# ZeayW/Multimodal-fusion-based-Pre-routing-Timing-Prediction-

Hardware: AMD Instinct MI355X
Metric: train-step samples/sec (higher is better)
Workload: dtype bf16; 1 GPU; config B: 8 designs/step/GPU, 65536-node netlist, 64 levels, 256x256 tile, 1350 endpoints/design, UNet(max), bf16 operands / fp32 accumulate on the MFMA-bound contractions; U-Net activations and their gradients stored bf16, netlist tensors, statistics, parameters and gradients fp32; nodes=65536, levels=64, tile=256, endpoints_per_design=1350, cone_pruning=False, parallelism=dp1 (designs sharded, one all-reduce of the flat gradient per step), launch=one HIP graph replay per step (Adam inside)

## Files before the change

multimodal-fusion-based-pre-routing-timing-prediction-_amd/csrc/unet16_conv.hip:

```cpp
#include <type_traits>
#include "unet16.h"

namespace mmft {

struct U16PackDesc {
  const float* w;
  u16* out;
  int rows, K;
  int taps;
  int mode;
  int Rsrc, Ksrc;
};

__global__ void __launch_bounds__(256) u16_pack_kernel(const U16PackDesc* __restrict__ descs, long long* __restrict__ counters,
                                                       int ncounters, long long inc) {
  if (counters && blockIdx.x == 0 && blockIdx.y == 0 && (int)threadIdx.x < ncounters) counters[threadIdx.x] += inc;
  const U16PackDesc d = descs[blockIdx.y];
  const int mode = d.mode & 3, KW = (d.mode & 4) ? 8 : 4, G = KW / 4;
  const int KB = d.K / (4 * KW), MB = d.rows / 16;
  const long long items = (long long)MB * d.taps * KB * 64 * G;
  for (long long e = (long long)blockIdx.x * 256 + threadIdx.x; e < items; e += (long long)gridDim.x * 256) {
    const int g = (int)(e % G);
    const int lane = (int)((e / G) & 63);
    long long f = e / (64 * G);
    const int kb = (int)(f % KB);
    f /= KB;
    const int t = (int)(f % d.taps), mb = (int)(f / d.taps);
    const int r = lane & 15, q = lane >> 4;
    const int row = mb * 16 + r;
    float v[4];
#pragma unroll
    for (int j = 0; j < 4; ++j) {
      const int k = kb * 4 * KW + KW * q + 4 * g + j;
      float x = 0.f;
      if (row < d.Rsrc && k < d.Ksrc) {
        if (mode == 0) x = d.w[((long long)row * d.taps + t) * d.Ksrc + k];
        else if (mode == 1) x = d.w[((long long)k * d.taps + (d.taps - 1 - t)) * d.Rsrc + row];
        else x = d.w[(long long)k * d.Rsrc + row];
      }
      v[j] = x;
    }
    *reinterpret_cast<s16x4*>(d.out + e * 4) = pack_bf16x4(v[0], v[1], v[2], v[3]);
  }
}

typedef __bf16 u16_bf16x8 __attribute__((ext_vector_type(8)));
typedef short u16_s16x8 __attribute__((ext_vector_type(8)));

struct U16ConvArgs {
  const void* x;
  const u16* wpk;
  u16* y;
  float* stats;
  int N, H, W, CO;
  int tiles_x, tiles_y, tiles;
  const float* gamma;
  const float* beta;
  const float* rmean;
  const float* rvar;
  float eps;
  int lda;
  u16* pooled;
  int pool_mode;
};

template <int CI, int TH, int TW>
struct U16ConvCfg {
  static constexpr bool K32 = CI >= 32;
  static constexpr int XR = TH + 2, XC = TW + 2, PIX = CI + (K32 ? 16 : 8);
  static constexpr int XS_BYTES = XR * XC * PIX * 2;
  static constexpr int RED_BYTES = 4 * 2 * 32 * 4;
  static constexpr int LDS_BYTES = XS_BYTES + RED_BYTES;
};

template <int CI, int COB, int TH, int TW, bool RGB, bool EVAL = false>
__global__ void __launch_bounds__(256) u16_conv3x3_kernel(U16ConvArgs a) {
  using C = U16ConvCfg<CI, TH, TW>;
  constexpr int XR = C::XR, XC = C::XC, PIX = C::PIX, MB = COB / 16;
  constexpr bool K32 = C::K32;
  constexpr int KC = K32 ? 32 : 16, NCH = CI / KC;
  constexpr int STEPS = TH * TW / 16, SPR = TW / 16, SPW = STEPS / 4;
  static_assert(TW % 16 == 0 && CI % 16 == 0 && COB % 16 == 0 && STEPS % 4 == 0 && (!RGB || CI == 16), "granularity");
  static_assert(!EVAL || (SPR <= 4 && (4 / SPR) * SPW == TH && SPW % 2 == 0), "eval epilogue: a wave owns SPW consecutive rows");
  extern __shared__ __attribute__((aligned(16))) unsigned char smem[];
  u16* xs = reinterpret_cast<u16*>(smem);
  float* red = reinterpret_cast<float*>(smem + C::XS_BYTES);
  const int tid = threadIdx.x, lane = tid & 63, wave = tid >> 6;
  const int r = lane & 15, q = lane >> 4;
  const int mb0 = blockIdx.y * MB, co0 = mb0 * 16;
  const f32x4 zero = {0.f, 0.f, 0.f, 0.f};
  auto strip = [&](int s, int& row, int& c0) {
    if constexpr (EVAL) {
      row = (wave / SPR) * SPW + s;
      c0 = (wave % SPR) * 16;
    } else {
      const int st = wave + 4 * s;
      row = st / SPR;
      c0 = (st % SPR) * 16;
    }
  };

  typedef typename std::conditional<K32, u16_bf16x8, s16x4>::type wfrag_t;
  wfrag_t wf[9][MB];
  auto load_weights = [&](int ch) {
#pragma unroll
    for (int t = 0; t < 9; ++t)
#pragma unroll
      for (int m = 0; m < MB; ++m)
        wf[t][m] = *reinterpret_cast<const wfrag_t*>(a.wpk + ((((long long)(mb0 + m) * 9 + t) * NCH + ch) * 64 + lane) * (KC / 4));
  };
  if constexpr (NCH == 1) load_weights(0);

  constexpr int XG = RGB ? 1 : CI / 8, XI = XR * XC * XG, NX = (XI + 255) / 256;
  if constexpr (RGB) {
    for (int e = tid; e < XR * XC * PIX / 4; e += 256) reinterpret_cast<s16x4*>(xs)[e] = s16x4{0, 0, 0, 0};
    __syncthreads();
  }
  u32x4 xr[NX];
  auto request = [&](int tile) {
    const int tx = tile % a.tiles_x, ty = (tile / a.tiles_x) % a.tiles_y, img = tile / (a.tiles_x * a.tiles_y);
    const int x0 = tx * TW, y0 = ty * TH;
    const long long img0 = (long long)img * a.H;
#pragma unroll
    for (int k = 0; k < NX; ++k) {
      const int it = tid + k * 256;
      const int cg = it % XG, col = (it / XG) % XC, row = it / (XG * XC);
      const int yy = y0 - 1 + row, xx = x0 - 1 + col;
      const bool ok = it < XI && yy >= 0 && yy < a.H && xx >= 0 && xx < a.W;
      const long long pix = (img0 + (ok ? yy : y0)) * a.W + (ok ? xx : x0);
      u32x4 v = {0u, 0u, 0u, 0u};
      if constexpr (RGB) {
        const float* src = reinterpret_cast<const float*>(a.x) + pix * 3;
        const s16x4 p = pack_bf16x4(src[0], src[1], src[2], 0.f);
        const u32x2 pp = as_u32x2(p);
        v[0] = pp[0];
        v[1] = pp[1];
      } else {
        v = *reinterpret_cast<const u32x4*>(reinterpret_cast<const u16*>(a.x) + pix * CI + cg * 8);
      }
      const u32x4 z4 = {0u, 0u, 0u, 0u};
      xr[k] = ok ? v : z4;
    }
  };
  auto deposit = [&]() {
#pragma unroll
    for (int k = 0; k < NX; ++k) {
      const int it = tid + k * 256;
      if (it < XI) {
        if constexpr (RGB) {
          u32x2 p = {xr[k][0], xr[k][1]};
          *reinterpret_cast<u32x2*>(xs + it * PIX) = p;
        } else {
          *reinterpret_cast<u32x4*>(xs + (it / XG) * PIX + (it % XG) * 8) = xr[k];
        }
      }
    }
  };

  float sc[EVAL ? MB : 1][4], sh[EVAL ? MB : 1][4];
  if constexpr (EVAL) {
#pragma unroll
    for (int m = 0; m < MB; ++m)
#pragma unroll
      for (int j = 0; j < 4; ++j) {
        const int c = co0 + m * 16 + 4 * q + j;
        const float rv = a.rvar[c];
        sc[m][j] = bn_frozen_scale(a.gamma[c], rv, a.eps);
        sh[m][j] = __fmaf_rn(-a.rmean[c], sc[m][j], a.beta[c]);
      }
  }

  if ((int)blockIdx.x < a.tiles) request(blockIdx.x);
  for (int tile = blockIdx.x; tile < a.tiles; tile += gridDim.x) {
    deposit();
    __syncthreads();
    if (tile + (int)gridDim.x < a.tiles) request(tile + gridDim.x);
    const int tx = tile % a.tiles_x, ty = (tile / a.tiles_x) % a.tiles_y, img = tile / (a.tiles_x * a.tiles_y);
    const int x0 = tx * TW, y0 = ty * TH;
    f32x4 acc[SPW][MB];
#pragma unroll
    for (int s = 0; s < SPW; ++s)
#pragma unroll
      for (int m = 0; m < MB; ++m) acc[s][m] = zero;
#pragma unroll 1
    for (int ch = 0; ch < NCH; ++ch) {
      if constexpr (NCH > 1) load_weights(ch);
#pragma unroll
      for (int s = 0; s < SPW; ++s) {
        int row, c0;
        strip(s, row, c0);
#pragma unroll
        for (int ky = 0; ky < 3; ++ky)
#pragma unroll
          for (int kx = 0; kx < 3; ++kx)
          {
            const u16* xp = xs + ((row + ky) * XC + c0 + r + kx) * PIX + ch * KC + (KC / 4) * q;
            if constexpr (K32) {
              const u16_bf16x8 xf = *reinterpret_cast<const u16_bf16x8*>(xp);
#pragma unroll
              for (int m = 0; m < MB; ++m) acc[s][m] = __builtin_amdgcn_mfma_f32_16x16x32_bf16(wf[ky * 3 + kx][m], xf, acc[s][m], 0, 0, 0);
            } else {
              const s16x4 xf = *reinterpret_cast<const s16x4*>(xp);
#pragma unroll
              for (int m = 0; m < MB; ++m) acc[s][m] = mfma_bf16_k16(wf[ky * 3 + kx][m], xf, acc[s][m]);
            }
          }
      }
    }
    if constexpr (EVAL) {
      u32x2 pk[SPW][MB];
#pragma unroll
      for (int s = 0; s < SPW; ++s) {
        int row, c0;
        strip(s, row, c0);
        const int yy = y0 + row, xx = x0 + c0 + r;
        const bool valid = yy < a.H && xx < a.W;
        u16* out = a.y + (((long long)img * a.H + yy) * a.W + xx) * a.lda + co0;
#pragma unroll
        for (int m = 0; m < MB; ++m) {
          float v[4];
#pragma unroll
          for (int j = 0; j < 4; ++j) {
            const float t = bn_pre(acc[s][m][j], sc[m][j], sh[m][j]);
            v[j] = t > 0.f ? t : 0.f;
          }
          const s16x4 p4 = pack_bf16x4(v[0], v[1], v[2], v[3]);
          if (valid) *reinterpret_cast<s16x4*>(out + m * 16 + 4 * q) = p4;
          pk[s][m] = as_u32x2(p4);
        }
      }
      if (a.pooled) {
        const int H2 = a.H / 2, W2 = a.W / 2;
        int row0, c0;
        strip(0, row0, c0);
        const int xx = x0 + c0 + r;
#pragma unroll
        for (int s = 0; s < SPW; s += 2) {
          const int yy = y0 + row0 + s;
          const bool store = (r & 1) == 0 && yy < a.H && xx < a.W;
          u16* out = a.pooled + (((long long)img * H2 + yy / 2) * W2 + xx / 2) * a.CO + co0;
#pragma unroll
          for (int m = 0; m < MB; ++m) {
            u32x2 nb0, nb1;
#pragma unroll
            for (int i = 0; i < 2; ++i) {
              nb0[i] = __shfl_xor(pk[s][m][i], 1, 64);
              nb1[i] = __shfl_xor(pk[s + 1][m][i], 1, 64);
            }
            float f00[4], f01[4], f10[4], f11[4], o[4];
            unpack4(pk[s][m], f00);
            unpack4(nb0, f01);
            unpack4(pk[s + 1][m], f10);
            unpack4(nb1, f11);
#pragma unroll
            for (int j = 0; j < 4; ++j) {
              if (a.pool_mode == MMFT_POOL_MAX) o[j] = fmaxf(fmaxf(f00[j], f01[j]), fmaxf(f10[j], f11[j]));
              else o[j] = (((f00[j] + f01[j]) + f10[j]) + f11[j]) * 0.25f;
            }
            if (store) *reinterpret_cast<s16x4*>(out + m * 16 + 4 * q) = pack_bf16x4(o[0], o[1], o[2], o[3]);
          }
        }
      }
      __syncthreads();
      continue;
    }
    float sm[MB][4], sq[MB][4];
#pragma unroll
    for (int m = 0; m < MB; ++m)
#pragma unroll
      for (int j = 0; j < 4; ++j) sm[m][j] = sq[m][j] = 0.f;
#pragma unroll
    for (int s = 0; s < SPW; ++s) {
      int row, c0;
      strip(s, row, c0);
      const int yy = y0 + row, xx = x0 + c0 + r;
      const bool valid = yy < a.H && xx < a.W;
      u16* out = a.y + (((long long)img * a.H + yy) * a.W + xx) * a.CO + co0;
#pragma unroll
      for (int m = 0; m < MB; ++m) {
        const s16x4 pk = pack_bf16x4(acc[s][m]);
        if (valid) *reinterpret_cast<s16x4*>(out + m * 16 + 4 * q) = pk;
        if (a.stats) {
#pragma unroll
          for (int j = 0; j < 4; ++j) {
            const float v = valid ? bf2f((unsigned)(unsigned short)pk[j]) : 0.f;
            sm[m][j] += v;
            sq[m][j] = __fmaf_rn(v, v, sq[m][j]);
          }
        }
      }
    }
    if (a.stats) {
#pragma unroll
      for (int m = 0; m < MB; ++m)
#pragma unroll
        for (int j = 0; j < 4; ++j) {
          float s1 = sm[m][j], s2 = sq[m][j];
#pragma unroll
          for (int o = 1; o < 16; o <<= 1) {
            s1 += __shfl_xor(s1, o, 64);
            s2 += __shfl_xor(s2, o, 64);
          }
          if (r == 0) {
            red[(wave * 2 + 0) * 32 + m * 16 + 4 * q + j] = s1;
            red[(wave * 2 + 1) * 32 + m * 16 + 4 * q + j] = s2;
          }
        }
    }
    __syncthreads();
    if (a.stats && tid < 2 * COB) {
      const int which = tid / COB, c = tid % COB;
      const float t = ((red[(0 * 2 + which) * 32 + c] + red[(1 * 2 + which) * 32 + c]) + red[(2 * 2 + which) * 32 + c]) +
                      red[(3 * 2 + which) * 32 + c];
      a.stats[((long long)tile * 2 + which) * a.CO + co0 + c] = t;
    }
  }
}

struct U16WgradArgs {
  const void* x;
  const u16* dy;
  float* slabs;
  int N, H, W, CI, CO;
  int tiles_x, tiles_y, tiles;
};

constexpr int u16_tr_pitch(int ch) { return ch == 16 ? 16 : 48; }

template <int CIB, int COB, int TH, int TW>
struct U16WgradCfg {
  static constexpr int XR = TH + 2, XC = TW + 2, PIXX = u16_tr_pitch(CIB), PIXD = u16_tr_pitch(COB);
  static constexpr int XS_BYTES = XR * XC * PIXX * 2, DS_BYTES = TH * TW * PIXD * 2;
  static constexpr int LDS_BYTES = XS_BYTES + DS_BYTES;
};

typedef __attribute__((address_space(3))) s16x4 lds_s16x4;
__device__ __forceinline__ s16x4 lds_tr_read(const u16* p) {
  return __builtin_amdgcn_ds_read_tr16_b64_v4i16((lds_s16x4*)p);
}

__device__ __forceinline__ u16_bf16x8 join8(s16x4 lo, s16x4 hi) {
  u16_s16x8 v = {lo[0], lo[1], lo[2], lo[3], hi[0], hi[1], hi[2], hi[3]};
  return __builtin_bit_cast(u16_bf16x8, v);
}

template <int CIB, int COB, int TH, int TW, bool RGB>
__global__ void __launch_bounds__(256) u16_conv3x3_wgrad_kernel(U16WgradArgs a) {
  using C = U16WgradCfg<CIB, COB, TH, TW>;
  constexpr int XR = C::XR, XC = C::XC, PIXX = C::PIXX, PIXD = C::PIXD, CB = CIB / 16, MB = COB / 16;
  constexpr int UNITS = 9 * CB, UM = (UNITS + 3) / 4;
  constexpr int SPT = TW / 32, STEPS = TH * SPT;
  static_assert(TW % 32 == 0 && CIB % 16 == 0 && COB % 16 == 0 && (!RGB || CIB == 16), "granularity");
  extern __shared__ __attribute__((aligned(16))) unsigned char smem[];
  u16* xs = reinterpret_cast<u16*>(smem);
  u16* ds = reinterpret_cast<u16*>(smem + C::XS_BYTES);
  const int tid = threadIdx.x, lane = tid & 63, wave = __builtin_amdgcn_readfirstlane(tid >> 6);
  const int nci = RGB ? 1 : a.CI / CIB;
  const int co0 = ((int)blockIdx.y / nci) * COB, ci0 = ((int)blockIdx.y % nci) * CIB;
  const f32x4 zero = {0.f, 0.f, 0.f, 0.f};
  const int tr_pix = 4 * (lane >> 4) + ((lane >> 2) & 3), tr_ch = 4 * (lane & 3);

  f32x4 acc[MB][UM];
#pragma unroll
  for (int m = 0; m < MB; ++m)
#pragma unroll
    for (int i = 0; i < UM; ++i) acc[m][i] = zero;

  constexpr int XG = RGB ? 1 : CIB / 8, XI = XR * XC * XG, NX = (XI + 255) / 256;
  constexpr int DG = COB / 8, DI = TH * TW * DG, ND = (DI + 255) / 256;
  if constexpr (RGB) {
    for (int e = tid; e < XR * XC * PIXX / 4; e += 256) reinterpret_cast<s16x4*>(xs)[e] = s16x4{0, 0, 0, 0};
    __syncthreads();
  }
  u32x4 xr[NX], dr[ND];
  auto request = [&](int tile) {
    const int tx = tile % a.tiles_x, ty = (tile / a.tiles_x) % a.tiles_y, img = tile / (a.tiles_x * a.tiles_y);
    const int x0 = tx * TW, y0 = ty * TH;
    const long long img0 = (long long)img * a.H;
    const u32x4 z4 = {0u, 0u, 0u, 0u};
#pragma unroll
    for (int k = 0; k < NX; ++k) {
      const int it = tid + k * 256;
      const int cg = it % XG, col = (it / XG) % XC, row = it / (XG * XC);
      const int yy = y0 - 1 + row, xx = x0 - 1 + col;
      const bool ok = it < XI && yy >= 0 && yy < a.H && xx >= 0 && xx < a.W;
      const long long pix = (img0 + (ok ? yy : y0)) * a.W + (ok ? xx : x0);
      u32x4 v = z4;
      if constexpr (RGB) {
        const float* src = reinterpret_cast<const float*>(a.x) + pix * 3;
        const u32x2 pp = as_u32x2(pack_bf16x4(src[0], src[1], src[2], 0.f));
        v[0] = pp[0];
        v[1] = pp[1];
      } else {
        v = *reinterpret_cast<const u32x4*>(reinterpret_cast<const u16*>(a.x) + pix * a.CI + ci0 + cg * 8);
      }
      xr[k] = ok ? v : z4;
    }
#pragma unroll
    for (int k = 0; k < ND; ++k) {
      const int it = tid + k * 256;
      const int cg = it % DG, col = (it / DG) % TW, row = it / (DG * TW);
      const int yy = y0 + row, xx = x0 + col;
      const bool ok = it < DI && yy < a.H && xx < a.W;
      const long long pix = (img0 + (ok ? yy : y0)) * a.W + (ok ? xx : x0);
      const u32x4 v = *reinterpret_cast<const u32x4*>(a.dy + pix * a.CO + co0 + cg * 8);
      dr[k] = ok ? v : z4;
    }
  };
  auto deposit = [&]() {
#pragma unroll
    for (int k = 0; k < NX; ++k) {
      const int it = tid + k * 256;
      if (it < XI) {
        if constexpr (RGB) {
          u32x2 p = {xr[k][0], xr[k][1]};
          *reinterpret_cast<u32x2*>(xs + it * PIXX) = p;
        } else {
          *reinterpret_cast<u32x4*>(xs + (it / XG) * PIXX + (it % XG) * 8) = xr[k];
        }
      }
    }
#pragma unroll
    for (int k = 0; k < ND; ++k) {
      const int it = tid + k * 256;
      if (it < DI) *reinterpret_cast<u32x4*>(ds + (it / DG) * PIXD + (it % DG) * 8) = dr[k];
    }
  };

  if ((int)blockIdx.x < a.tiles) request(blockIdx.x);
  for (int tile = blockIdx.x; tile < a.tiles; tile += gridDim.x) {
    deposit();
    __syncthreads();
    if (tile + (int)gridDim.x < a.tiles) request(tile + gridDim.x);
#pragma unroll 2
    for (int st = 0; st < STEPS; ++st) {
      const int row = st / SPT, c0 = (st % SPT) * 32;
      u16_bf16x8 af[MB];
      const u16* dbase = ds + (row * TW + c0 + tr_pix) * PIXD + tr_ch;
#pragma unroll
      for (int m = 0; m < MB; ++m) af[m] = join8(lds_tr_read(dbase + m * 16), lds_tr_read(dbase + 16 * PIXD + m * 16));
#pragma unroll
      for (int i = 0; i < UM; ++i) {
        const int u = wave + 4 * i;
        if (u < UNITS) {
          const int t = u / CB, c = u % CB, ky = t / 3, kx = t % 3;
          const u16* xb = xs + ((row + ky) * XC + c0 + kx + tr_pix) * PIXX + c * 16 + tr_ch;
          const u16_bf16x8 bfr = join8(lds_tr_read(xb), lds_tr_read(xb + 16 * PIXX));
#pragma unroll
          for (int m = 0; m < MB; ++m) acc[m][i] = __builtin_amdgcn_mfma_f32_16x16x32_bf16(af[m], bfr, acc[m][i], 0, 0, 0);
        }
      }
    }
    __syncthreads();
  }

  const int r = lane & 15, q = lane >> 4;
  const int CIs = RGB ? 3 : a.CI;
  float* out = a.slabs + (long long)blockIdx.x * ((long long)a.CO * 9 * CIs);
#pragma unroll
  for (int i = 0; i < UM; ++i) {
    const int u = wave + 4 * i;
    if (u < UNITS) {
      const int t = u / CB, c = u % CB;
#pragma unroll
      for (int m = 0; m < MB; ++m)
#pragma unroll
        for (int j = 0; j < 4; ++j) {
          const int co = co0 + m * 16 + 4 * q + j, ci = c * 16 + r;
          if (!RGB || ci < 3) out[((long long)co * 9 + t) * CIs + ci0 + ci] = acc[m][i][j];
        }
    }
  }
}

static inline void u16_tile_shape(int W, int* th, int* tw) {
  *tw = W >= 64 ? 64 : 32;
  *th = 256 / *tw;
}

template <int CI, int COB, int TH, int TW, bool RGB, bool EVAL = false>
static int u16_conv_launch_t(const U16ConvArgs& a, int grid_x, hipStream_t st, double flops, double bytes) {
  using C = U16ConvCfg<CI, TH, TW>;
  static DynLdsOnce once;
  int rc = ensure_dyn_lds(once, reinterpret_cast<const void*>(&u16_conv3x3_kernel<CI, COB, TH, TW, RGB, EVAL>), C::LDS_BYTES, "u16_conv3x3");
  if (rc) return rc;
  static char name[64];
  if (!name[0])
    snprintf(name, sizeof(name), EVAL ? "u16_conv3x3_eval_kernel<%d,%d,%dx%d%s>" : "u16_conv3x3_kernel<%d,%d,%dx%d%s>", RGB ? 3 : CI, COB,
             TH, TW, a.stats ? "" : "");
  MMFT_LAUNCH_LDS(name, flops, bytes, (u16_conv3x3_kernel<CI, COB, TH, TW, RGB, EVAL>), dim3(grid_x, a.CO / COB), dim3(256),
                  C::LDS_BYTES, st, a);
  return check_launch(EVAL ? "u16_conv3x3_eval" : "u16_conv3x3");
}

template <bool EVAL>
static int u16_conv_dispatch(U16ConvArgs& a, int rgb_f32, int Ci, hipStream_t st, double flops, double bytes) {
  int th, tw;
  u16_tile_shape(a.W, &th, &tw);
  a.tiles_x = (a.W + tw - 1) / tw;
  a.tiles_y = (a.H + th - 1) / th;
  a.tiles = a.N * a.tiles_x * a.tiles_y;
  const int cob = a.CO % 32 == 0 ? 32 : 16, gy = a.CO / cob;
  int cap = 2048 / gy;
  const int gx = a.tiles < cap ? a.tiles : cap;
#define U16_CONV(CIV, COBV, RGBV)                                                                           \
  (tw == 64 ? u16_conv_launch_t<CIV, COBV, 4, 64, RGBV, EVAL>(a, gx, st, flops, bytes)                      \
            : u16_conv_launch_t<CIV, COBV, 8, 32, RGBV, EVAL>(a, gx, st, flops, bytes))
  if (rgb_f32) return U16_CONV(16, 16, true);
  if (cob == 16) {
    if (Ci == 16) return U16_CONV(16, 16, false);
    if (Ci == 32) return U16_CONV(32, 16, false);
    if (Ci == 64) return U16_CONV(64, 16, false);
    return U16_CONV(128, 16, false);
  }
  if (Ci == 16) return U16_CONV(16, 32, false);
  if (Ci == 32) return U16_CONV(32, 32, false);
  if (Ci == 64) return U16_CONV(64, 32, false);
  return U16_CONV(128, 32, false);
#undef U16_CONV
}

template <int CIB, int COB, int TH, int TW, bool RGB>
static int u16_wgrad_launch_t(const U16WgradArgs& a, int grid_x, int grid_y, hipStream_t st, double flops, double bytes) {
  using C = U16WgradCfg<CIB, COB, TH, TW>;
  static DynLdsOnce once;
  int rc = ensure_dyn_lds(once, reinterpret_cast<const void*>(&u16_conv3x3_wgrad_kernel<CIB, COB, TH, TW, RGB>), C::LDS_BYTES,
                          "u16_conv3x3_wgrad");
  if (rc) return rc;
  static char name[64];
  if (!name[0]) snprintf(name, sizeof(name), "u16_conv3x3_wgrad_kernel<%d,%d,%dx%d>", RGB ? 3 : CIB, COB, TH, TW);
  MMFT_LAUNCH_LDS(name, flops, bytes, (u16_conv3x3_wgrad_kernel<CIB, COB, TH, TW, RGB>), dim3(grid_x, grid_y),
                  dim3(256), C::LDS_BYTES, st, a);
  return check_launch("u16_conv3x3_wgrad");
}

static inline bool u16_channels_ok(int c) { return c == 16 || c == 32 || c == 64 || c == 128; }

static inline int u16_wgrad_grid_x(int tiles, int grid_y) {
  int cap = 512 / grid_y;
  if (cap < 8) cap = 8;
  int g = (tiles + 1) / 2;
  if (g > cap) g = cap;
  return g < 1 ? 1 : g;
}

}

using namespace mmft;

extern "C" {

int mmft_u16_pack_weights(const void* descs, int n, long long max_frag_lanes, long long* counters, int ncounters, long long inc,
                          int device, void* stream) {
  MMFT_REQUIRE(descs && n > 0 && max_frag_lanes > 0 && ncounters >= 0 && ncounters <= 256, "u16_pack_weights: bad arguments");
  DeviceGuard dg(device);
  long long gx = (max_frag_lanes + 255) / 256;
  if (gx > 64) gx = 64;
  MMFT_LAUNCH("u16_pack_kernel", 0.0, 6.0 * 4.0 * max_frag_lanes * n / 2, u16_pack_kernel, dim3((int)gx, n), dim3(256), (hipStream_t)stream,
              reinterpret_cast<const U16PackDesc*>(descs), counters, ncounters, inc);
  return check_launch("u16_pack_weights");
}

int mmft_u16_pack_desc_bytes(void) { return (int)sizeof(U16PackDesc); }

int mmft_u16_conv_tiles(int N, int H, int W, int* per_image) {
  int th, tw;
  u16_tile_shape(W, &th, &tw);
  const int t = ((H + th - 1) / th) * ((W + tw - 1) / tw);
  if (per_image) *per_image = t;
  return N * t;
}

int mmft_u16_conv3x3(const void* x, int rgb_f32, const void* wpk, void* y, float* stats, int N, int H, int W, int Ci, int Co,
                     int device, void* stream) {
  MMFT_REQUIRE(x && wpk && y && N > 0 && H > 0 && W > 0, "u16_conv3x3: bad arguments");
  MMFT_REQUIRE(u16_channels_ok(Co) && (rgb_f32 ? (Ci == 3 && Co == 16) : u16_channels_ok(Ci)),
               "u16_conv3x3: channels must be 16 / 32 / 64 / 128 (or the 3 -> 16 RGB layer)");
  MMFT_REQUIRE(aligned16(x) && aligned16(wpk) && aligned16(y), "u16_conv3x3: 16-byte alignment");
  DeviceGuard dg(device);
  U16ConvArgs a{x, reinterpret_cast<const u16*>(wpk), reinterpret_cast<u16*>(y), stats, N, H, W, Co};
  const double flops = 2.0 * N * H * W * Co * 9.0 * Ci;
  const double bytes = (rgb_f32 ? 4.0 : 2.0) * N * H * W * Ci + 2.0 * N * H * W * Co + 2.0 * Co * 9 * Ci;
  return u16_conv_dispatch<false>(a, rgb_f32, Ci, (hipStream_t)stream, flops, bytes);
}

int mmft_u16_conv3x3_eval(const void* x, int rgb_f32, const void* wpk, const float* gamma, const float* beta, const float* running_mean,
                          const float* running_var, float eps, void* a, int lda, void* pooled, int pool_mode, int N, int H, int W,
                          int Ci, int Co, int device, void* stream) {
  MMFT_REQUIRE(x && wpk && a && gamma && beta && running_mean && running_var && N > 0 && H > 0 && W > 0 && eps >= 0.f,
               "u16_conv3x3_eval: bad arguments");
  MMFT_REQUIRE(u16_channels_ok(Co) && (rgb_f32 ? (Ci == 3 && Co == 16) : u16_channels_ok(Ci)),
               "u16_conv3x3_eval: channels must be 16 / 32 / 64 / 128 (or the 3 -> 16 RGB layer)");
  MMFT_REQUIRE(lda >= Co && lda % 8 == 0, "u16_conv3x3_eval: the pixel pitch must hold Co channels and be a multiple of 8");
  MMFT_REQUIRE(!pooled || (H % 2 == 0 && W % 2 == 0 && (pool_mode == MMFT_POOL_MAX || pool_mode == MMFT_POOL_AVG)),
               "u16_conv3x3_eval: pooling needs even H, W and a pooling mode");
  MMFT_REQUIRE(aligned16(x) && aligned16(wpk) && aligned16(a) && (!pooled || aligned16(pooled)), "u16_conv3x3_eval: 16-byte alignment");
  DeviceGuard dg(device);
  U16ConvArgs p{x, reinterpret_cast<const u16*>(wpk), reinterpret_cast<u16*>(a), nullptr, N, H, W, Co};
  p.gamma = gamma;
  p.beta = beta;
  p.rmean = running_mean;
  p.rvar = running_var;
  p.eps = eps;
  p.lda = lda;
  p.pooled = reinterpret_cast<u16*>(pooled);
  p.pool_mode = pool_mode;
  const double flops = 2.0 * N * H * W * Co * 9.0 * Ci;
  const double bytes = (rgb_f32 ? 4.0 : 2.0) * N * H * W * Ci + 2.0 * N * H * W * Co * (pooled ? 1.25 : 1.0) + 2.0 * Co * 9 * Ci;
  return u16_conv_dispatch<true>(p, rgb_f32, Ci, (hipStream_t)stream, flops, bytes);
}

long long mmft_u16_conv3x3_wgrad_workspace_bytes(int N, int H, int W, int Ci, int Co) {
  int th, tw;
  u16_tile_shape(W, &th, &tw);
  const int tiles = N * ((H + th - 1) / th) * ((W + tw - 1) / tw);
  const int cib = Ci == 3 ? 16 : (Ci % 32 == 0 ? 32 : 16), cob = Co % 32 == 0 ? 32 : 16;
  const int gy = (Co / cob) * (Ci == 3 ? 1 : Ci / cib);
  return (long long)u16_wgrad_grid_x(tiles, gy) * Co * 9 * Ci * 4;
}

int mmft_u16_conv3x3_wgrad_slabs(int N, int H, int W, int Ci, int Co) {
  return (int)(mmft_u16_conv3x3_wgrad_workspace_bytes(N, H, W, Ci, Co) / ((long long)Co * 9 * Ci * 4));
}

int mmft_u16_conv3x3_wgrad(const void* x, int rgb_f32, const void* dy, float* dw, int accumulate, int N, int H, int W, int Ci,
                           int Co, float* workspace, long long workspace_bytes, int device, void* stream) {
  MMFT_REQUIRE(x && dy && N > 0 && H > 0 && W > 0, "u16_conv3x3_wgrad: bad arguments");
  MMFT_REQUIRE(u16_channels_ok(Co) && (rgb_f32 ? (Ci == 3 && Co == 16) : u16_channels_ok(Ci)),
               "u16_conv3x3_wgrad: channels must be 16 / 32 / 64 / 128 (or the 3 -> 16 RGB layer)");
  MMFT_REQUIRE(workspace && workspace_bytes >= mmft_u16_conv3x3_wgrad_workspace_bytes(N, H, W, Ci, Co) && aligned16(workspace) &&
                   aligned16(x) && aligned16(dy) && (!dw || aligned16(dw)),
               "u16_conv3x3_wgrad: workspace too small or operands not 16-byte aligned");
  DeviceGuard dg(device);
  hipStream_t st = (hipStream_t)stream;
  int th, tw;
  u16_tile_shape(W, &th, &tw);
  U16WgradArgs a{x, reinterpret_cast<const u16*>(dy), workspace, N, H, W, Ci, Co, (W + tw - 1) / tw, (H + th - 1) / th, 0};
  a.tiles = N * a.tiles_x * a.tiles_y;
  const int cib = rgb_f32 ? 16 : (Ci % 32 == 0 ? 32 : 16), cob = Co % 32 == 0 ? 32 : 16;
  const int gy = (Co / cob) * (rgb_f32 ? 1 : Ci / cib);
  const int gx = u16_wgrad_grid_x(a.tiles, gy);
  const double flops = 2.0 * N * H * W * Co * 9.0 * Ci;
  const double bytes = (rgb_f32 ? 4.0 : 2.0) * N * H * W * Ci + 2.0 * N * H * W * Co;
  int rc;
#define U16_WG(CIBV, COBV, RGBV)                                                                            \
  (tw == 64 ? u16_wgrad_launch_t<CIBV, COBV, 4, 64, RGBV>(a, gx, gy, st, flops, bytes)                      \
            : u16_wgrad_launch_t<CIBV, COBV, 8, 32, RGBV>(a, gx, gy, st, flops, bytes))
  if (rgb_f32) rc = U16_WG(16, 16, true);
  else if (cib == 16 && cob == 16) rc = U16_WG(16, 16, false);
  else if (cib == 16) rc = U16_WG(16, 32, false);
  else if (cob == 16) rc = U16_WG(32, 16, false);
  else rc = U16_WG(32, 32, false);
#undef U16_WG
  if (rc || !dw) return rc;
  return launch_slab_reduce(workspace, gx, (long long)Co * 9 * Ci, dw, accumulate, st);
}

}
```

multimodal-fusion-based-pre-routing-timing-prediction-_amd/mmft/unet16.py:

```python
import ctypes
import functools
import math
import weakref

import torch
from torch import nn

from . import gradsink, lib, ops

ENABLED = True


def supported(net, x, frozen_stats=False):
    if not ENABLED or net.bilinear or x.dim() != 4 or x.shape[1] != 3 or x.dtype != torch.float32 or not x.is_cuda:
        return False
    if x.shape[0] > 1 and not net.inc.per_sample_stats and not frozen_stats:
        return False
    H, W = x.shape[2], x.shape[3]
    return H % 8 == 0 and W % 32 == 0 and H >= 8


def _params(net):
    ps = net.__dict__.get('_u16_param_list')
    if ps is None:
        ps = net.__dict__['_u16_param_list'] = list(net.parameters())
    return ps


def _layers(net):
    cached = net.__dict__.get('_u16_layers')
    if cached is not None:
        return cached
    net.__dict__['_u16_layers'] = out = _layers_uncached(net)
    return out


def _layers_uncached(net):
    dcs = [net.inc, net.down1.maxpool_conv[1], net.down2.maxpool_conv[1], net.down3.maxpool_conv[1],
           net.up1.conv, net.up2.conv, net.up3.conv]
    out = []
    for dc in dcs:
        s = dc.double_conv
        out.append((s[0], s[1]))
        out.append((s[3], s[4]))
    return out


class _PackDesc(ctypes.Structure):
    _fields_ = [('w', ctypes.c_void_p), ('out', ctypes.c_void_p), ('rows', ctypes.c_int), ('K', ctypes.c_int), ('taps', ctypes.c_int),
                ('mode', ctypes.c_int), ('Rsrc', ctypes.c_int), ('Ksrc', ctypes.c_int)]


def _pad16(n):
    return (n + 15) // 16 * 16


def pack_table(entries, device):
    assert lib.query('mmft_u16_pack_desc_bytes') == ctypes.sizeof(_PackDesc)
    total = sum(rows * K * taps for _, _, rows, K, taps, _, _, _ in entries)
    buf = torch.empty(total, dtype=torch.bfloat16, device=device)
    descs = (_PackDesc * len(entries))()
    offs, off, lanes = {}, 0, 0
    for j, (name, p, rows, K, taps, mode, Rsrc, Ksrc) in enumerate(entries):
        descs[j] = _PackDesc(p.data_ptr(), buf.data_ptr() + off * 2, rows, K, taps, mode, Rsrc, Ksrc)
        offs[name] = off
        off += rows * K * taps
        lanes = max(lanes, rows * K * taps // 4)
    table = torch.frombuffer(bytearray(bytes(descs)), dtype=torch.uint8).to(device)
    return buf, table, offs, lanes


def pack_run(buf, table, n, lanes, counters=None, inc=0):
    dev, st = lib.stream_args(buf)
    lib.call('mmft_u16_pack_weights', table, n, lanes, counters, counters.numel() if counters is not None else 0, int(inc), dev, st)


def conv_pack_entries(name, weight, backward=False):
    Co, Ci = weight.shape[0], weight.shape[1]
    if not ops.is_nhwc(weight):
        raise RuntimeError('unet16: Conv2d weights must be stored channels_last ([Co][3][3][Ci] memory)')
    if backward:
        return (name, weight, Ci, Co, 9, 1 + (4 if Co >= 32 else 0), Ci, Co)
    return (name, weight, Co, _pad16(Ci), 9, 0 + (4 if Ci >= 32 else 0), Co, Ci)


def convt_pack_entries(name, weight, backward=False):
    Ci, Co = weight.shape[0], weight.shape[1]
    if not weight.permute(2, 3, 1, 0).is_contiguous():
        raise RuntimeError('unet16: ConvTranspose2d weights must be stored in (a,b,co,ci) memory order')
    if backward:
        return (name, weight, Ci, 4 * Co, 1, 2, Ci, 4 * Co)
    return (name, weight, 4 * Co, Ci, 1, 0, 4 * Co, Ci)


class _Packs:

    def __init__(self, net, device):
        self.key = None
        self.device = device

    def _build(self, net):
        entries = []
        for i, (cv, _) in enumerate(_layers(net)):
            entries.append(conv_pack_entries('f%d' % i, cv.weight))
            if i > 0:
                entries.append(conv_pack_entries('b%d' % i, cv.weight, backward=True))
        for k, up in enumerate([net.up1.up, net.up2.up, net.up3.up]):
            entries.append(convt_pack_entries('tf%d' % k, up.weight))
            entries.append(convt_pack_entries('tb%d' % k, up.weight, backward=True))
        self.buf, self.descs, self.off, self.lanes = pack_table(entries, self.device)
        self.n = len(entries)

    def ensure(self, net):
        key = tuple(p.data_ptr() for p in _params(net))
        if key != self.key:
            self._build(net)
            self.key = key

    def refresh(self, net, counters=None, inc=0):
        self.ensure(net)
        pack_run(self.buf, self.descs, self.n, self.lanes, counters, inc)

    def ptr(self, name):
        return self.buf.data_ptr() + self.off[name] * 2


def _arena(sizes, dtype, device, align=128):
    off, table = 0, {}
    for name, n in sizes:
        table[name] = (off, n)
        off += (n + align - 1) // align * align
    buf = torch.empty(max(off, 1), dtype=dtype, device=device)
    return buf, {k: buf[o:o + n] for k, (o, n) in table.items()}


class _Sink:

    def __init__(self, param, mem_shape, to_logical):
        self.rec = gradsink.of(param)
        self.to_logical = to_logical
        view = None
        if self.rec is not None:
            mem, _ = gradsink._memory_order(self.rec[0])
            if mem is not None and mem.numel() == math.prod(mem_shape):
                view = mem.reshape(mem_shape)
        self.direct = view is not None
        if self.direct:
            self.out, self.accumulate = view, not gradsink.fresh(self.rec)
        else:
            self.out, self.accumulate = torch.empty(mem_shape, dtype=torch.float32, device=param.device), False

    def done(self):
        if self.direct:
            if not self.accumulate:
                gradsink.taken(self.rec)
            return None
        return self.to_logical(self.out)


def _geometry(N, H, W):
    lv = [(H >> k, W >> k) for k in range(4)]
    P = [N * h * w for h, w in lv]
    return lv, P


_CONV = {1: (3, 16, 0, 'x'), 2: (16, 16, 0, 'a1'), 3: (16, 32, 1, 'p1'), 4: (32, 32, 1, 'a3'), 5: (32, 64, 2, 'p2'),
         6: (64, 64, 2, 'a5'), 7: (64, 128, 3, 'p3'), 8: (128, 128, 3, 'a7'), 9: (128, 64, 2, 'cat1'), 10: (64, 64, 2, 'a9'),
         11: (64, 32, 1, 'cat2'), 12: (32, 32, 1, 'a11'), 13: (32, 16, 0, 'cat3'), 14: (16, 16, 0, 'a13')}
_ACT = {1: ('a1', 16, None), 2: ('cat3', 32, 'p1'), 3: ('a3', 32, None), 4: ('cat2', 64, 'p2'), 5: ('a5', 64, None),
        6: ('cat1', 128, 'p3'), 7: ('a7', 128, None), 8: ('a8', 128, None), 9: ('a9', 64, None), 10: ('a10', 64, None),
        11: ('a11', 32, None), 12: ('a12', 32, None), 13: ('a13', 16, None), 14: ('a14', 16, None)}
_UP = {0: (128, 'a8', 'cat1', 64, 3), 1: (64, 'a10', 'cat2', 32, 2), 2: (32, 'a12', 'cat3', 16, 1)}


@functools.lru_cache(maxsize=16)
def _fwd_sizes(N, H, W):
    lv, P = _geometry(N, H, W)
    sizes = [('z%d' % i, P[_CONV[i][2]] * _CONV[i][1]) for i in range(1, 15)]
    sizes += [('a1', P[0] * 16), ('cat3', P[0] * 32), ('p1', P[1] * 16), ('a3', P[1] * 32), ('cat2', P[1] * 64), ('p2', P[2] * 32),
              ('a5', P[2] * 64), ('cat1', P[2] * 128), ('p3', P[3] * 64), ('a7', P[3] * 128), ('a8', P[3] * 128), ('a9', P[2] * 64),
              ('a10', P[2] * 64), ('a11', P[1] * 32), ('a12', P[1] * 32), ('a13', P[0] * 16), ('a14', P[0] * 16)]
    per_img = ctypes.c_int(0)
    tiles0 = lib.load().mmft_u16_conv_tiles(N, lv[0][0], lv[0][1], ctypes.byref(per_img))
    fsizes = [('stats', tiles0 * 2 * 128)] + [('bnp%d' % i, 5 * N * _CONV[i][1]) for i in range(1, 15)]
    return sizes, fsizes


@functools.lru_cache(maxsize=16)
def _bwd_sizes(N, H, W):
    lv, P = _geometry(N, H, W)
    sizes = [('g%d' % i, P[_CONV[i][2]] * _CONV[i][1]) for i in range(1, 15)] + [('dz%d' % i, P[_CONV[i][2]] * _CONV[i][1]) for i in range(1, 15)]
    sizes += [('gcat3', P[0] * 32), ('gcat2', P[1] * 64), ('gcat1', P[2] * 128), ('gp1', P[1] * 16), ('gp2', P[2] * 32), ('gp3', P[3] * 64)]
    q = lib.query
    ws_bytes = max([q('mmft_u16_outconv_bwd_workspace_bytes', N, H, W)] +
                   [q('mmft_u16_bn_bwd_workspace_bytes', N, lv[_CONV[i][2]][0] * lv[_CONV[i][2]][1], _CONV[i][1]) for i in range(1, 15)] +
                   [q('mmft_u16_conv3x3_wgrad_workspace_bytes', N, lv[_CONV[i][2]][0], lv[_CONV[i][2]][1], _CONV[i][0], _CONV[i][1])
                    for i in range(1, 15)] +
                   [q('mmft_u16_convt_wgrad_workspace_bytes', N, lv[u[4]][0], lv[u[4]][1], u[0]) for u in _UP.values()])
    return sizes, ws_bytes


BATCH_REDUCE = True


@functools.lru_cache(maxsize=16)
def _slab_sizes(N, H, W):
    lv, _ = _geometry(N, H, W)
    q = lib.query
    sizes = [('sw%d' % i, q('mmft_u16_conv3x3_wgrad_workspace_bytes', N, lv[_CONV[i][2]][0], lv[_CONV[i][2]][1], _CONV[i][0], _CONV[i][1]) // 4)
             for i in range(1, 15)]
    sizes += [('st%d' % k, q('mmft_u16_convt_wgrad_workspace_bytes', N, lv[u[4]][0], lv[u[4]][1], u[0]) // 4) for k, u in _UP.items()]
    sizes += [('so', q('mmft_u16_outconv_bwd_workspace_bytes', N, H, W) // 4)]
    return sizes


def _run_forward(net, xn, pool_mode, packs, T, F, out, geom):
    N, H, W = geom
    dev, st = lib.stream_args(out)
    lv, _ = _geometry(N, H, W)
    convs = _layers(net)
    ups = [net.up1.up, net.up2.up, net.up3.up]
    packs.refresh(net, counters=net._batch_counters(), inc=N if net.inc.per_sample_stats else 1)
    per_img = ctypes.c_int(0)
    for i in range(1, 15):
        Ci, Co, l, inp = _CONV[i]
        h, w = lv[l]
        cv, bn = convs[i - 1]
        xin = xn if inp == 'x' else T[inp]
        lib.load().mmft_u16_conv_tiles(N, h, w, ctypes.byref(per_img))
        lib.call('mmft_u16_conv3x3', xin, 1 if inp == 'x' else 0, packs.ptr('f%d' % (i - 1)), T['z%d' % i], F['stats'], N, h, w,
                 Ci, Co, dev, st)
        lib.call('mmft_u16_bn_finalize', F['stats'], per_img.value, N, Co, h * w, float(bn.eps), bn.weight.detach(), bn.bias.detach(),
                 F['bnp%d' % i], dev, st)
        abuf_name, lda, pooled = _ACT[i]
        lib.call('mmft_u16_bn_apply', T['z%d' % i], F['bnp%d' % i], T[abuf_name], lda, T[pooled] if pooled else None, N, h, w, Co,
                 pool_mode, float(bn.momentum), bn.running_mean, bn.running_var, dev, st)
        for k, (uCi, uin, cat, coff, ul) in _UP.items():
            if uin == abuf_name:
                up = ups[k]
                uh, uw = lv[ul]
                lib.call('mmft_u16_convt_fwd', T[uin], packs.ptr('tf%d' % k), up.bias.detach() if up.bias is not None else None,
                         T[cat].data_ptr() + coff * 2, 2 * (uCi // 2), N, uh, uw, uCi, dev, st)
    oc = net.outc.conv[0]
    lib.call('mmft_u16_outconv_fwd', T['a14'], oc.weight.detach(), oc.bias.detach() if oc.bias is not None else None, out, N, H, W,
             pool_mode, dev, st)


@functools.lru_cache(maxsize=16)
def _eval_sizes(N, H, W):
    return [(name, n) for name, n in _fwd_sizes(N, H, W)[0] if not name.startswith('z')]


def _run_forward_eval(net, xn, pool_mode, packs, T, out, geom):
    N, H, W = geom
    dev, st = lib.stream_args(out)
    lv, _ = _geometry(N, H, W)
    convs = _layers(net)
    ups = [net.up1.up, net.up2.up, net.up3.up]
    packs.refresh(net)
    for i in range(1, 15):
        Ci, Co, l, inp = _CONV[i]
        h, w = lv[l]
        _, bn = convs[i - 1]
        abuf_name, lda, pooled = _ACT[i]
        lib.call('mmft_u16_conv3x3_eval', xn if inp == 'x' else T[inp], 1 if inp == 'x' else 0, packs.ptr('f%d' % (i - 1)),
                 bn.weight.detach(), bn.bias.detach(), bn.running_mean, bn.running_var, float(bn.eps), T[abuf_name], lda,
                 T[pooled] if pooled else None, pool_mode, N, h, w, Ci, Co, dev, st)
        for k, (uCi, uin, cat, coff, ul) in _UP.items():
            if uin == abuf_name:
                up = ups[k]
                uh, uw = lv[ul]
                lib.call('mmft_u16_convt_fwd', T[uin], packs.ptr('tf%d' % k), up.bias.detach() if up.bias is not None else None,
                         T[cat].data_ptr() + coff * 2, 2 * (uCi // 2), N, uh, uw, uCi, dev, st)
    oc = net.outc.conv[0]
    lib.call('mmft_u16_outconv_fwd', T['a14'], oc.weight.detach(), oc.bias.detach() if oc.bias is not None else None, out, N, H, W,
             pool_mode, dev, st)


def _forward_eval(net, x):
    N, _, H, W = x.shape
    if not all(bn.affine for _, bn in _layers(net)):
        raise NotImplementedError('unet16: BatchNorm2d without affine is not on the reference path')
    pooling = net.down1.maxpool_conv[0]
    pool_mode = ops.POOL_MAX if isinstance(pooling, nn.MaxPool2d) else ops.POOL_AVG
    packs = net.__dict__.get('_u16_packs')
    if packs is None or packs.device != x.device:
        packs = net.__dict__['_u16_packs'] = _Packs(net, x.device)
    xn = ops.to_nhwc(x.detach())
    abuf, T = _arena(_eval_sizes(N, H, W), torch.bfloat16, x.device)
    out = torch.empty((N, 1, H // 2, W // 2), dtype=torch.float32, device=x.device)
    _run_forward_eval(net, xn, pool_mode, packs, T, out, (N, H, W))
    return out, pool_mode, packs, xn, abuf, T


def unet_forward_eval(net, x):
    return _forward_eval(net, x)[0]


_EVAL_SHAPE = {'a1': (0, 16), 'cat3': (0, 32), 'p1': (1, 16), 'a3': (1, 32), 'cat2': (1, 64), 'p2': (2, 32), 'a5': (2, 64),
               'cat1': (2, 128), 'p3': (3, 64), 'a7': (3, 128), 'a8': (3, 128), 'a9': (2, 64), 'a10': (2, 64), 'a11': (1, 32),
               'a12': (1, 32), 'a13': (0, 16), 'a14': (0, 16)}


def _param_state(net):
    ps = _params(net)
    return tuple(p.data_ptr() for p in ps), tuple(p._version for p in ps), gradsink.param_epoch()


class EvalTape:

    def __init__(self, net, geom, pool_mode, packs, xn, abuf, T):
        self.net, self.geom, self.pool_mode, self.packs, self.xn, self.arena, self.T = net, geom, pool_mode, packs, xn, abuf, T
        self.pack_buf, self.state = packs.buf, _param_state(net)
# ... 295 lines not shown
```

Baseline: 2573 designs/s.

## Add double-buffered weight prefetch and deep-layer dispatch for bf16 U-Net 3x3 convs

Adds a WPF variant of the 3x3 conv kernel for layers with 64 or more input channels. It double-buffers the per-chunk weight fragments in registers, batches the LDS strip reads ahead of the MFMA groups using sched barriers, and requests a block's own tile at the start of each iteration instead of the next one. A separate deep-layer dispatch halves the tile height when the grid would under-fill the CUs, and only uses COB=32 when there are enough tiles. It also adds a runtime switch and grid-cap tuning API, with an environment variable to disable the path. In exchange, register pressure rises (possibly two waves per SIMD limited by launch bounds) and the input-tile prefetch that used to overlap compute across tiles is lost.

```diff
diff --git a/include/mmft_u16_tune.h b/include/mmft_u16_tune.h
--- /dev/null
+++ b/include/mmft_u16_tune.h
@@ -0,0 +1,17 @@
+#ifndef MMFT_U16_TUNE_H
+#define MMFT_U16_TUNE_H
+
+#include "mmft.h"
+
+#ifdef __cplusplus
+extern "C" {
+#endif
+
+int mmft_u16_conv_tune(int deep, int grid_cap);
+
+long long mmft_u16_conv_tuning(void);
+
+#ifdef __cplusplus
+}
+#endif
+#endif
diff --git a/multimodal-fusion-based-pre-routing-timing-prediction-_amd/csrc/unet16_conv.hip b/multimodal-fusion-based-pre-routing-timing-prediction-_amd/csrc/unet16_conv.hip
--- a/multimodal-fusion-based-pre-routing-timing-prediction-_amd/csrc/unet16_conv.hip
+++ b/multimodal-fusion-based-pre-routing-timing-prediction-_amd/csrc/unet16_conv.hip
@@ -1,5 +1,8 @@
+#include <atomic>
+#include <cstdlib>
 #include <type_traits>
 #include "unet16.h"
+#include "../../include/mmft_u16_tune.h"
 
 namespace mmft {
 
@@ -73,8 +76,8 @@
   static constexpr int LDS_BYTES = XS_BYTES + RED_BYTES;
 };
 
-template <int CI, int COB, int TH, int TW, bool RGB, bool EVAL = false>
-__global__ void __launch_bounds__(256) u16_conv3x3_kernel(U16ConvArgs a) {
+template <int CI, int COB, int TH, int TW, bool RGB, bool EVAL = false, bool WPF = false>
+__global__ void __launch_bounds__(256, (WPF && 2 * U16ConvCfg<CI, TH, TW>::LDS_BYTES <= 160 * 1024) ? 2 : 1) u16_conv3x3_kernel(U16ConvArgs a) {
   using C = U16ConvCfg<CI, TH, TW>;
   constexpr int XR = C::XR, XC = C::XC, PIX = C::PIX, MB = COB / 16;
   constexpr bool K32 = C::K32;
@@ -82,6 +85,7 @@
   constexpr int STEPS = TH * TW / 16, SPR = TW / 16, SPW = STEPS / 4;
   static_assert(TW % 16 == 0 && CI % 16 == 0 && COB % 16 == 0 && STEPS % 4 == 0 && (!RGB || CI == 16), "granularity");
   static_assert(!EVAL || (SPR <= 4 && (4 / SPR) * SPW == TH && SPW % 2 == 0), "eval epilogue: a wave owns SPW consecutive rows");
+  static_assert(!WPF || (K32 && NCH >= 2 && NCH % 2 == 0 && !EVAL), "weight prefetch: an even number of 32-channel chunks, two register sets");
   extern __shared__ __attribute__((aligned(16))) unsigned char smem[];
   u16* xs = reinterpret_cast<u16*>(smem);
   float* red = reinterpret_cast<float*>(smem + C::XS_BYTES);
@@ -109,6 +113,16 @@
       for (int m = 0; m < MB; ++m)
         wf[t][m] = *reinterpret_cast<const wfrag_t*>(a.wpk + ((((long long)(mb0 + m) * 9 + t) * NCH + ch) * 64 + lane) * (KC / 4));
   };
+  wfrag_t wf1[WPF ? 9 : 1][MB];
+  typedef __attribute__((address_space(1))) wfrag_t global_wfrag_t;
+  auto prefetch_weights = [&](wfrag_t (&w)[9][MB], int ch) {
+    const char* wch = reinterpret_cast<const char*>(a.wpk + (((long long)mb0 * 9 * NCH + ch) * 64 + lane) * (KC / 4));
+    asm volatile("" : "+v"(wch));
+#pragma unroll
+    for (int t = 0; t < 9; ++t)
+#pragma unroll
+      for (int m = 0; m < MB; ++m) w[t][m] = *(const global_wfrag_t*)(wch + (m * 9 + t) * NCH * 64 * (KC / 4) * 2);
+  };
   if constexpr (NCH == 1) load_weights(0);
 
   constexpr int XG = RGB ? 1 : CI / 8, XI = XR * XC * XG, NX = (XI + 255) / 256;
@@ -170,11 +184,17 @@
       }
   }
 
-  if ((int)blockIdx.x < a.tiles) request(blockIdx.x);
+  if constexpr (!WPF)
+    if ((int)blockIdx.x < a.tiles) request(blockIdx.x);
   for (int tile = blockIdx.x; tile < a.tiles; tile += gridDim.x) {
+    if constexpr (WPF) {
+      prefetch_weights(wf, 0);
+      request(tile);
+    }
     deposit();
     __syncthreads();
-    if (tile + (int)gridDim.x < a.tiles) request(tile + gridDim.x);
+    if constexpr (!WPF)
+      if (tile + (int)gridDim.x < a.tiles) request(tile + gridDim.x);
     const int tx = tile % a.tiles_x, ty = (tile / a.tiles_x) % a.tiles_y, img = tile / (a.tiles_x * a.tiles_y);
     const int x0 = tx * TW, y0 = ty * TH;
     f32x4 acc[SPW][MB];
@@ -182,6 +202,46 @@
     for (int s = 0; s < SPW; ++s)
 #pragma unroll
       for (int m = 0; m < MB; ++m) acc[s][m] = zero;
+    auto read_strip = [&](u16_bf16x8 (&xf)[9], int s, int ch) {
+      int row, c0;
+      strip(s, row, c0);
+#pragma unroll
+      for (int t = 0; t < 9; ++t)
+        xf[t] = *reinterpret_cast<const u16_bf16x8*>(xs + ((row + t / 3) * XC + c0 + r + t % 3) * PIX + ch * KC + (KC / 4) * q);
+    };
+    auto mfma_strip = [&](const wfrag_t (&w)[9][MB], const u16_bf16x8 (&xf)[9], int s) {
+#pragma unroll
+      for (int t = 0; t < 9; ++t)
+#pragma unroll
+        for (int m = 0; m < MB; ++m)
+          if constexpr (K32) acc[s][m] = __builtin_amdgcn_mfma_f32_16x16x32_bf16(w[t][m], xf[t], acc[s][m], 0, 0, 0);
+    };
+    auto chunk_batched = [&](const wfrag_t (&w)[9][MB], int ch) {
+      u16_bf16x8 xa[9], xb[9];
+      read_strip(xa, 0, ch);
+#pragma unroll
+      for (int s = 0; s < SPW; s += 2) {
+        if (s + 1 < SPW) read_strip(xb, s + 1, ch);
+        __builtin_amdgcn_sched_barrier(0);
+        mfma_strip(w, xa, s);
+        if (s + 1 < SPW) {
+          if (s + 2 < SPW) read_strip(xa, s + 2, ch);
+          __builtin_amdgcn_sched_barrier(0);
+          mfma_strip(w, xb, s + 1);
+        }
+      }
+    };
+    if constexpr (WPF) {
+#pragma unroll 1
+      for (int ch = 0; ch < NCH; ch += 2) {
+        prefetch_weights(wf1, ch + 1);
+        __builtin_amdgcn_sched_barrier(0);
+        chunk_batched(wf, ch);
+        if (ch + 2 < NCH) prefetch_weights(wf, ch + 2);
+        __builtin_amdgcn_sched_barrier(0);
+        chunk_batched(wf1, ch + 1);
+      }
+    } else {
 #pragma unroll 1
     for (int ch = 0; ch < NCH; ++ch) {
       if constexpr (NCH > 1) load_weights(ch);
@@ -206,6 +266,7 @@
             }
           }
       }
+    }
     }
     if constexpr (EVAL) {
       u32x2 pk[SPW][MB];
@@ -478,30 +539,72 @@
   *th = 256 / *tw;
 }
 
-template <int CI, int COB, int TH, int TW, bool RGB, bool EVAL = false>
+template <int CI, int COB, int TH, int TW, bool RGB, bool EVAL = false, bool WPF = false>
 static int u16_conv_launch_t(const U16ConvArgs& a, int grid_x, hipStream_t st, double flops, double bytes) {
   using C = U16ConvCfg<CI, TH, TW>;
   static DynLdsOnce once;
-  int rc = ensure_dyn_lds(once, reinterpret_cast<const void*>(&u16_conv3x3_kernel<CI, COB, TH, TW, RGB, EVAL>), C::LDS_BYTES, "u16_conv3x3");
+  int rc = ensure_dyn_lds(once, reinterpret_cast<const void*>(&u16_conv3x3_kernel<CI, COB, TH, TW, RGB, EVAL, WPF>), C::LDS_BYTES, "u16_conv3x3");
   if (rc) return rc;
   static char name[64];
   if (!name[0])
     snprintf(name, sizeof(name), EVAL ? "u16_conv3x3_eval_kernel<%d,%d,%dx%d%s>" : "u16_conv3x3_kernel<%d,%d,%dx%d%s>", RGB ? 3 : CI, COB,
-             TH, TW, a.stats ? "" : "");
-  MMFT_LAUNCH_LDS(name, flops, bytes, (u16_conv3x3_kernel<CI, COB, TH, TW, RGB, EVAL>), dim3(grid_x, a.CO / COB), dim3(256),
+             TH, TW, WPF ? ",pf" : "");
+  MMFT_LAUNCH_LDS(name, flops, bytes, (u16_conv3x3_kernel<CI, COB, TH, TW, RGB, EVAL, WPF>), dim3(grid_x, a.CO / COB), dim3(256),
                   C::LDS_BYTES, st, a);
   return check_launch(EVAL ? "u16_conv3x3_eval" : "u16_conv3x3");
 }
 
+#ifndef MMFT_U16_DEEP_WPF
+#define MMFT_U16_DEEP_WPF true
+#endif
+constexpr bool U16_DEEP_WPF = MMFT_U16_DEEP_WPF;
+constexpr int U16_CUS = 256;
+constexpr int U16_GRID_CAP = 2048;
+static std::atomic<int> g_u16_deep{-1}, g_u16_grid_cap{U16_GRID_CAP};
+static int u16_deep_conv() {
+  int v = g_u16_deep.load(std::memory_order_relaxed);
+  if (v < 0) {
+    const char* e = getenv("MMFT_U16_DEEP_CONV");
+    v = (e && atoi(e) == 0) ? 0 : 1;
+    g_u16_deep.store(v, std::memory_order_relaxed);
+  }
+  return v;
+}
+
+static int u16_conv_dispatch_deep(U16ConvArgs& a, int Ci, hipStream_t st, double flops, double bytes) {
+  int th, tw;
+  u16_tile_shape(a.W, &th, &tw);
+  a.tiles_x = (a.W + tw - 1) / tw;
+  const long long full = (long long)a.N * a.tiles_x * ((a.H + th - 1) / th);
+  const bool half = a.stats == nullptr && full * (a.CO / 16) < 2 * U16_CUS;
+  if (half) th /= 2;
+  a.tiles_y = (a.H + th - 1) / th;
+  a.tiles = a.N * a.tiles_x * a.tiles_y;
+  const int cob = (Ci == 128 && !half && (long long)a.tiles * (a.CO / 32) >= U16_CUS) ? 32 : 16, gy = a.CO / cob;
+  int cap = g_u16_grid_cap.load(std::memory_order_relaxed) / gy;
+  if (cap < 1) cap = 1;
+  const int gx = a.tiles < cap ? a.tiles : cap;
+#define U16_DEEP(CIV, COBV, THV, TWV) u16_conv_launch_t<CIV, COBV, THV, TWV, false, false, U16_DEEP_WPF>(a, gx, st, flops, bytes)
+#define U16_DEEP16(CIV)                                                                                             \
+  (tw == 64 ? (half ? U16_DEEP(CIV, 16, 2, 64) : U16_DEEP(CIV, 16, 4, 64)) : (half ? U16_DEEP(CIV, 16, 4, 32) : U16_DEEP(CIV, 16, 8, 32)))
+  if (Ci == 64) return U16_DEEP16(64);
+  if (cob == 16) return U16_DEEP16(128);
+  return tw == 64 ? U16_DEEP(128, 32, 4, 64) : U16_DEEP(128, 32, 8, 32);
+#undef U16_DEEP16
+#undef U16_DEEP
+}
+
 template <bool EVAL>
 static int u16_conv_dispatch(U16ConvArgs& a, int rgb_f32, int Ci, hipStream_t st, double flops, double bytes) {
+  if (!EVAL && !rgb_f32 && Ci >= 64 && u16_deep_conv()) return u16_conv_dispatch_deep(a, Ci, st, flops, bytes);
   int th, tw;
   u16_tile_shape(a.W, &th, &tw);
   a.tiles_x = (a.W + tw - 1) / tw;
   a.tiles_y = (a.H + th - 1) / th;
   a.tiles = a.N * a.tiles_x * a.tiles_y;
   const int cob = a.CO % 32 == 0 ? 32 : 16, gy = a.CO / cob;
-  int cap = 2048 / gy;
+  int cap = g_u16_grid_cap.load(std::memory_order_relaxed) / gy;
+  if (cap < 1) cap = 1;
   const int gx = a.tiles < cap ? a.tiles : cap;
 #define U16_CONV(CIV, COBV, RGBV)                                                                           \
   (tw == 64 ? u16_conv_launch_t<CIV, COBV, 4, 64, RGBV, EVAL>(a, gx, st, flops, bytes)                      \
@@ -570,6 +673,15 @@
   if (per_image) *per_image = t;
   return N * t;
 }
+
+int mmft_u16_conv_tune(int deep, int grid_cap) {
+  MMFT_REQUIRE(deep >= -1 && deep <= 1 && grid_cap >= -1, "u16_conv_tune: deep is -1 / 0 / 1, grid_cap -1, 0 or a number of workgroups");
+  if (deep >= 0) g_u16_deep.store(deep, std::memory_order_relaxed);
+  if (grid_cap >= 0) g_u16_grid_cap.store(grid_cap ? grid_cap : U16_GRID_CAP, std::memory_order_relaxed);
+  return 0;
+}
+
+long long mmft_u16_conv_tuning(void) { return ((long long)g_u16_grid_cap.load(std::memory_order_relaxed) << 1) | u16_deep_conv(); }
 
 int mmft_u16_conv3x3(const void* x, int rgb_f32, const void* wpk, void* y, float* stats, int N, int H, int W, int Ci, int Co,
                      int device, void* stream) {
diff --git a/multimodal-fusion-based-pre-routing-timing-prediction-_amd/mmft/unet16.py b/multimodal-fusion-based-pre-routing-timing-prediction-_amd/mmft/unet16.py
--- a/multimodal-fusion-based-pre-routing-timing-prediction-_amd/mmft/unet16.py
+++ b/multimodal-fusion-based-pre-routing-timing-prediction-_amd/mmft/unet16.py
@@ -1,3 +1,4 @@
+import contextlib
 import ctypes
 import functools
 import math
@@ -9,6 +10,18 @@
 from . import gradsink, lib, ops
 
 ENABLED = True
+
+abi = lib.Header('mmft_u16_tune.h')
+
+
+@contextlib.contextmanager
+def conv_tuning(deep=None, grid_cap=None):
+    prev = abi('mmft_u16_conv_tuning')
+    abi('mmft_u16_conv_tune', -1 if deep is None else int(bool(deep)), -1 if grid_cap is None else int(grid_cap))
+    try:
+        yield
+    finally:
+        abi('mmft_u16_conv_tune', prev & 1, prev >> 1)
 
 
 def supported(net, x, frozen_stats=False):
```

Result: faster. 2626 designs/s, median of 4 (+2.0%).
